# g1mv/density

Measured on NVIDIA H100. Metric: chameleon_encode_input_GBps, higher is better.
Workload: dtype u32

## Files before the change

density_b200/_lib.py:

```python
import ctypes
import os

_HERE = os.path.dirname(os.path.abspath(__file__))
SO_PATH = os.environ.get("DENSITY_B200_SO") or os.path.join(_HERE, "libdensity_b200.so")

_c_u8p = ctypes.c_void_p
_SIGS = {
    **{f"{a}_{op}": (ctypes.c_size_t, [_c_u8p, ctypes.c_size_t, _c_u8p, ctypes.c_size_t])
       for a in ("chameleon", "cheetah", "lion") for op in ("encode", "decode")},
    **{f"{a}_safe_encode_buffer_size": (ctypes.c_size_t, [ctypes.c_size_t]) for a in ("chameleon", "cheetah", "lion")},
    "density_b200_encode_device": (ctypes.c_int, [ctypes.c_int, _c_u8p, ctypes.c_size_t, _c_u8p, ctypes.c_size_t, ctypes.c_void_p, ctypes.c_void_p]),
    "density_b200_decode_device": (ctypes.c_int, [ctypes.c_int, _c_u8p, ctypes.c_size_t, _c_u8p, ctypes.c_size_t, ctypes.c_void_p, ctypes.c_void_p]),
    "density_b200_encode_device_path": (ctypes.c_int, [ctypes.c_int, _c_u8p, ctypes.c_size_t, _c_u8p, ctypes.c_size_t, ctypes.c_void_p, ctypes.c_void_p, ctypes.c_int]),
    "density_b200_decode_device_path": (ctypes.c_int, [ctypes.c_int, _c_u8p, ctypes.c_size_t, _c_u8p, ctypes.c_size_t, ctypes.c_void_p, ctypes.c_void_p, ctypes.c_int]),
    "density_b200_shard_create": (ctypes.c_void_p, []),
    "density_b200_shard_destroy": (None, [ctypes.c_void_p]),
    "density_b200_shard_phase1": (ctypes.c_int, [ctypes.c_void_p, _c_u8p, ctypes.c_size_t, ctypes.c_int, ctypes.c_void_p, ctypes.c_void_p]),
    "density_b200_shard_phase2": (ctypes.c_int, [ctypes.c_void_p, ctypes.c_void_p, _c_u8p, ctypes.c_size_t, ctypes.c_void_p, ctypes.c_void_p, ctypes.c_void_p]),
    "density_b200_sharded_unique_id": (ctypes.c_int, [ctypes.c_void_p]),
    "density_b200_sharded_create": (ctypes.c_void_p, [ctypes.c_void_p, ctypes.c_int, ctypes.c_int]),
    "density_b200_sharded_destroy": (None, [ctypes.c_void_p]),
    "density_b200_encode_sharded": (ctypes.c_int, [ctypes.c_void_p, _c_u8p, ctypes.c_size_t, _c_u8p, ctypes.c_size_t, ctypes.c_void_p, ctypes.c_void_p,
                                                   ctypes.c_void_p, ctypes.c_int, _c_u8p, ctypes.c_size_t, ctypes.c_void_p]),
    "density_b200_sharded_profile": (ctypes.c_int, [ctypes.c_void_p, ctypes.POINTER(ctypes.c_float)]),
# ... 23 lines not shown
    "density_b200_codec_create": (ctypes.c_void_p, [ctypes.c_int]),
    "density_b200_codec_destroy": (None, [ctypes.c_void_p]),
    "density_b200_codec_clear_state": (ctypes.c_int, [ctypes.c_void_p]),
    "density_b200_codec_encode": (ctypes.c_size_t, [ctypes.c_void_p, _c_u8p, ctypes.c_size_t, _c_u8p, ctypes.c_size_t]),
    "density_b200_codec_decode": (ctypes.c_size_t, [ctypes.c_void_p, _c_u8p, ctypes.c_size_t, _c_u8p, ctypes.c_size_t]),
    "density_b200_table_init": (ctypes.c_int, [ctypes.c_void_p, ctypes.c_void_p]),
    "density_b200_table_fold": (ctypes.c_int, [ctypes.c_void_p, ctypes.c_void_p, ctypes.c_void_p]),
    "density_b200_profile_enable": (None, [ctypes.c_int]),
    "density_b200_profile_get": (ctypes.c_int, [ctypes.POINTER(ctypes.c_float)]),
    "density_b200_last_error": (ctypes.c_char_p, []),
    "density_b200_kernel_launches": (ctypes.c_uint64, []),
    "density_b200_last_encode_was_fast": (ctypes.c_int, []),
    "density_b200_decode_status": (ctypes.c_int, [ctypes.POINTER(ctypes.c_uint64)]),
    "density_b200_cheetah_decode_rounds": (ctypes.c_int, [ctypes.POINTER(ctypes.c_uint32)]),
    "density_b200_encode_status": (ctypes.c_int, [ctypes.POINTER(ctypes.c_uint64)]),
    "density_b200_test_set_stage_rounds": (None, [ctypes.c_int]),
    "density_b200_prot_debug": (ctypes.c_int, [ctypes.POINTER(ctypes.c_uint64)]),
    "density_b200_shutdown": (None, []),
    "density_b200_version": (ctypes.c_char_p, []),
}
EXPORTED_SYMBOLS = tuple(sorted(_SIGS))

_lib = None


class DensityB200Error(RuntimeError):
    pass


def load():
# ... 18 lines not shown
```

density_b200/csrc/api.cu:

```cuda
#include "../../include/density_b200.h"
#include "common.cuh"
#include "encode_internal.cuh"

#include <dlfcn.h>

#include <atomic>
#include <condition_variable>
#include <cstdio>
#include <cstring>
#include <deque>
#include <mutex>
#include <string>
#include <thread>
#include <vector>

namespace dns {

static thread_local std::string g_last_error;
static std::atomic<uint64_t> g_launches{0};

static void set_error(const char* what, cudaError_t e) {
    char buf[512];
    snprintf(buf, sizeof buf, "%s: %s (%s)", what, cudaGetErrorString(e), cudaGetErrorName(e));
    g_last_error = buf;
// ... 137 lines not shown
struct DeviceCtx {
    int dev = -1;
    int num_sms = 0;
    bool ready = false;
    cudaStream_t stream = nullptr;
    cudaStream_t h2d_stream = nullptr, d2h_stream = nullptr;
    DevBuf ws, stage_in, stage_out, pipe_tables, dec_tables;
    DevBuf chee_tables[2][3];
    uint32_t chee_epoch = 0;
    uint64_t* h_sizes = nullptr;
    cudaEvent_t ev_h2d[2] = {nullptr, nullptr};
    PinRing ring_in, ring_out;
    uint64_t* d_size = nullptr;
    uint64_t* h_size = nullptr;
    ChamLayout layout{};
    int last_was_chameleon_fastpath_capable = 0;
    bool profile = false;
    static constexpr int PROF_RING = 64;
    cudaEvent_t ev[PROF_RING][4] = {};
    uint64_t prof_count = 0;
    const void* last_cl_status = nullptr;
    cudaEvent_t ws_free = nullptr;
    bool ws_free_recorded = false;
    std::mutex mu;
};

constexpr int MAX_DEVICES = 64;
static DeviceCtx g_ctx[MAX_DEVICES];
static std::mutex g_ctx_mu;

// ... 61 lines not shown
static int encode_device_locked_impl(DeviceCtx* c, int alg, const uint8_t* d_in, size_t n, uint8_t* d_out, size_t cap,
                                     uint64_t* d_out_size, cudaStream_t stream, int path) {
    uint64_t launches = 0;
    cudaError_t e;
    const bool aligned = !(reinterpret_cast<uintptr_t>(d_in) & 3) && !(reinterpret_cast<uintptr_t>(d_out) & 1);
    if (alg == ALG_CHAMELEON && path != 3 && aligned) {
        ChamLayout L;
        size_t need = cham_workspace_bytes(n, c->num_sms, &L);
        e = c->ws.ensure(need, stream);
        if (e != cudaSuccess) { set_error("workspace cudaMalloc", e); return DENSITY_B200_ECUDA; }
        c->layout = L;
        if (path == 2) {
            e = cham_encode_protected_only(d_in, n, c->ws.p, L, d_out, cap, d_out_size, stream, &launches);
        } else {
            const uint32_t nruns = cham_pick_runs(n, c->num_sms);
            cudaEvent_t* ev = nullptr;
            if (c->profile) {
                ev = c->ev[c->prof_count % DeviceCtx::PROF_RING];
                for (int i = 0; i < 4; ++i) if (!ev[i]) cudaEventCreate(&ev[i]);
            }
            e = cham_encode_phase1(d_in, n, c->ws.p, L, nruns, nullptr, stream, &launches, ev);
            if (e == cudaSuccess && path == 4)
                e = cham_encode_phase2_blocking(d_in, n, c->ws.p, L, nruns, d_out, cap, d_out_size, 12, stream, &launches);
            else if (e == cudaSuccess)
                e = cham_encode_phase2(d_in, n, c->ws.p, L, nruns, nullptr, d_out, cap, d_out_size, path == 0, false, stream, &launches, ev);
            if (ev != nullptr && e == cudaSuccess) c->prof_count++;
        }
        c->last_was_chameleon_fastpath_capable = (path != 2);
    } else if ((alg == ALG_CHEETAH || alg == ALG_LION) && path != 3 && !(reinterpret_cast<uintptr_t>(d_in) & 3) && !(reinterpret_cast<uintptr_t>(d_out) & 1)) {
        const size_t pw = (chee_workspace_bytes(n, c->num_sms) + 255) & ~(size_t)255;
// ... 1074 lines not shown
    if (cudaDeviceSynchronize() != cudaSuccess) return 0;
    if (cudaMemcpy(&st, c->ws.p + c->layout.status, sizeof st, cudaMemcpyDeviceToHost) != cudaSuccess) return 0;
    return st.nonquiet ? 0 : 1;
}

int density_b200_encode_status(uint64_t* out6) {
    DeviceCtx* c = current_ctx();
    if (!c || !c->ws.p) return DENSITY_B200_EARG;
    std::lock_guard<std::mutex> lk(c->mu);
    Status st;
    if (cudaDeviceSynchronize() != cudaSuccess || cudaMemcpy(&st, c->ws.p + c->layout.status, sizeof st, cudaMemcpyDeviceToHost) != cudaSuccess) return DENSITY_B200_ECUDA;
    out6[0] = st.out_bytes; out6[1] = st.nonquiet; out6[2] = st.error; out6[3] = st.first_nonquiet_block; out6[4] = st.converged; out6[5] = st.iter_changed;
    return DENSITY_B200_OK;
}

void density_b200_shutdown(void) {
    std::lock_guard<std::mutex> lk(g_ctx_mu);
    int cur = -1;
    cudaGetDevice(&cur);
    for (int d = 0; d < MAX_DEVICES; ++d) {
        DeviceCtx& c = g_ctx[d];
        if (!c.ready) continue;
        cudaSetDevice(d);
        c.ws.release(); c.stage_in.release(); c.stage_out.release(); c.dec_tables.release(); for (int a2 = 0; a2 < 2; ++a2) for (int rg = 0; rg < 3; ++rg) c.chee_tables[a2][rg].release();
        c.chee_epoch = 0;
        if (c.d_size) cudaFree(c.d_size);
        if (c.h_size) cudaFreeHost(c.h_size);
        if (c.stream) cudaStreamDestroy(c.stream);
        if (c.ws_free) { cudaEventDestroy(c.ws_free); c.ws_free = nullptr; c.ws_free_recorded = false; }
        if (c.h2d_stream) cudaStreamDestroy(c.h2d_stream);
// ... 32 lines not shown
```

density_b200/csrc/chameleon_encode.cu:

```cuda
#include <cstdio>
#include "common.cuh"
#include "encode_internal.cuh"

namespace dns {
namespace cham {

constexpr int TILE_Q = 4096;
__device__ __forceinline__ bool bit_test(const uint32_t* bm, uint32_t i) { return (bm[i >> 5] >> (i & 31)) & 1u; }

constexpr int F6_THREADS = 512, F6_QPT = 8;
constexpr int F6_NW = F6_THREADS / 32, F6_WQ = 32 * F6_QPT;
static_assert(F6_THREADS * F6_QPT == TILE_Q, "tile geometry");
constexpr int F6_MB_SLOTS = 4096, F6_MB_CAP = 4;
constexpr int F6_SEC_SLOTS = 64, F6_SEC_CAP = 16;
#ifdef DNS_PHASE_TIMING
__device__ long long g_f6_ph[8];
#define F6_PH(k) { if (threadIdx.x == 0 && blockIdx.x == 77) { long long tn = clock64(); g_f6_ph[k] += tn - f6_tprev; f6_tprev = tn; } }
#define F6_PH_DECL long long f6_tprev = clock64();
#else
#define F6_PH(k)
#define F6_PH_DECL
#endif
constexpr uint32_t F6_TOUCHED = 1u << 12, F6_DROPPED = 1u << 13;
struct Flag6Smem {
// ... 334 lines not shown
        const uint32_t v = S.tab[i];
        const uint32_t tch = (v != 0 || bit_test(S.vbit, i)) ? 0x10000u : 0u;
        final_tab[(size_t)run * 65536 + i] = v | tch;
    }
    if (tid == 0) unres_count[run] = S.unres_count < 65536u ? S.unres_count : 65536u;
#ifdef DNS_PHASE_TIMING
    if (tid == 0 && run == 77 && ntile_run) { const long long nt = ntile_run;
        printf("f6 run %u tiles %lld cycles/tile: A %lld B %lld C+deposit %lld D+S4 %lld  overflow tiles %lld dirty/tile %lld\n", run, nt, g_f6_ph[0] / nt, g_f6_ph[1] / nt,
               g_f6_ph[2] / nt, g_f6_ph[3] / nt, g_f6_ph[6], g_f6_ph[7] / nt);
        for (int k = 0; k < 8; ++k) g_f6_ph[k] = 0; }
#endif
}

__device__ __forceinline__ bool gate_open(const Status* g) { return !g || (g->nonquiet && !g->converged); }

__global__ void cham_carry_scan(const uint32_t* __restrict__ final_tab, const uint32_t* __restrict__ init, int init_untouched,
                                uint32_t nruns, uint32_t* __restrict__ carry, uint32_t* __restrict__ table_out,
                                const Status* __restrict__ gate = nullptr) {
    if (!gate_open(gate)) return;
    uint32_t hb = blockIdx.x * blockDim.x + threadIdx.x;
    if (hb >= 65536) return;
    uint32_t c = init ? init[hb] : ((hb == 0 && !init_untouched) ? 0x10000u : 0u);
    for (uint32_t r = 0; r < nruns; ++r) {
        if (carry) carry[(size_t)r * 65536 + hb] = c;
        uint32_t v = final_tab[(size_t)r * 65536 + hb];
        if (v & 0x10000u) c = v;
    }
    if (table_out) table_out[hb] = c;
}

__global__ void cham_resolve(const uint2* __restrict__ unres, const uint32_t* __restrict__ unres_count,
                             const uint32_t* __restrict__ carry, uint32_t tiles_total, uint32_t nruns,
                             uint32_t* __restrict__ sigw_g, const Status* __restrict__ gate = nullptr) {
    if (!gate_open(gate)) return;
    const uint32_t run = blockIdx.y;
    const uint32_t n = unres_count[run];
    const uint64_t run_q0 = ((uint64_t)run * tiles_total / nruns) * TILE_Q;
    for (uint32_t i = blockIdx.x * blockDim.x + threadIdx.x; i < n; i += gridDim.x * blockDim.x) {
        uint2 e = unres[(size_t)run * 65536 + i];
        uint32_t c = carry[(size_t)run * 65536 + (e.y & 0xFFFFu)];
        if ((c & 0x10000u) && (c & 0xFFFFu) == (e.y >> 16)) {
            uint64_t gq = run_q0 + e.x;
            atomicOr(&sigw_g[gq >> 5], 1u << (gq & 31));
        }
    }
}

struct ProtSmem {
    uint16_t tab[65536];
    uint32_t vbit[2048];
};

__global__ void __launch_bounds__(1024, 1)
cham_protected_pass(const uint32_t* __restrict__ in, uint64_t nbytes, const Status* __restrict__ status, int only_if_nonquiet,
                    uint32_t* __restrict__ sigw_g, uint8_t* __restrict__ copymap) {
    if (only_if_nonquiet && !(status->nonquiet && !status->converged)) return;
    extern __shared__ __align__(16) unsigned char smem_raw[];
    ProtSmem& S = *reinterpret_cast<ProtSmem*>(smem_raw);
// ... 270 lines not shown
        for (uint64_t b = gtid; b < nblocks; b += gsz) cm_old[b] = __ldcg(&cm_new[b]);
    grid_barrier(bar, gridDim.x, epoch);
    if (gtid == 0 && converged) st->converged = 1;
}

__device__ __forceinline__ uint32_t block_out_bytes(uint64_t b, uint64_t nbytes, uint32_t hits, bool copied) {
    const uint64_t boff = b * 256;
    const uint32_t blen = (uint32_t)((nbytes - boff < 256) ? (nbytes - boff) : 256);
    return copied ? blen : 8 + blen - 2 * hits;
}

__global__ void cham_tile_sizes(const uint32_t* __restrict__ sigw_g, const uint8_t* __restrict__ copymap, uint64_t nbytes,
                                uint64_t nblocks, uint32_t ntiles, int use_copymap_if_nonquiet, int check_quiet, int assume_prev_inc,
                                Status* __restrict__ status, uint32_t* __restrict__ tile_bytes) {
    const uint32_t lane = threadIdx.x & 31;
    const uint32_t tile = blockIdx.x * (blockDim.x >> 5) + (threadIdx.x >> 5);
    if (tile >= ntiles) return;
    if (use_copymap_if_nonquiet && !check_quiet && !status->nonquiet) return;
    const bool use_cm = copymap && (!use_copymap_if_nonquiet || status->nonquiet);
    uint32_t sum = 0, incm[2];
#pragma unroll
    for (int k = 0; k < 2; ++k) {
        const uint64_t b = (uint64_t)tile * 64 + k * 32 + lane;
        uint32_t sz = 0; bool inc = false;
        if (b < nblocks) {
            const bool copied = use_cm && copymap[b];
            const uint32_t hits = __popc(sigw_g[2 * b]) + __popc(sigw_g[2 * b + 1]);
            sz = block_out_bytes(b, nbytes, hits, copied);
            inc = !copied && sz >= 256 && (nbytes - b * 256 >= 256);
        }
        sum += sz;
        incm[k] = __ballot_sync(0xFFFFFFFFu, inc);
    }
#pragma unroll
    for (int d = 16; d; d >>= 1) sum += __shfl_xor_sync(0xFFFFFFFFu, sum, d);
    if (lane == 0) tile_bytes[tile] = sum;
    if (check_quiet && lane == 0) {
        bool prev = assume_prev_inc != 0;
        if (tile > 0) {
            const uint64_t b = (uint64_t)tile * 64 - 1;
            const uint32_t hits = __popc(sigw_g[2 * b]) + __popc(sigw_g[2 * b + 1]);
            prev = (8 + 256 - 2 * hits) >= 256;
        }
        const uint64_t m = ((uint64_t)incm[1] << 32) | incm[0];
        const uint64_t pairs = m & ((m << 1) | (prev ? 1ull : 0ull));
        if (pairs) {
            atomicOr(&status->nonquiet, 1u);
            atomicMin(&status->first_nonquiet_block, (unsigned long long)tile * 64 + (__ffsll((long long)pairs) - 1));
        }
    }
}

constexpr int SCAN_T = 1024;
constexpr int SCAN_PER = 4;
constexpr int SCAN_G = SCAN_T * SCAN_PER;

__device__ __forceinline__ uint64_t block_exclusive_scan_u64(uint64_t v, uint64_t* s_warp, uint64_t* total) {
    const uint32_t lane = threadIdx.x & 31, warp = threadIdx.x >> 5;
    uint64_t incl = v;
#pragma unroll
    for (int d = 1; d < 32; d <<= 1) { uint64_t u = __shfl_up_sync(0xFFFFFFFFu, incl, d); if (lane >= (uint32_t)d) incl += u; }
    if (lane == 31) s_warp[warp] = incl;
    __syncthreads();
// ... 255 lines not shown
        if (w[2]) bad = 1;
        if (w[3]) { if (prev_inc && w[0]) bad = 1; prev_inc = w[1]; }
        if (d_sizes) d_sizes[r] = off;
        off += (uint64_t)w[4] | ((uint64_t)w[5] << 32);
    }
    if (d_sizes) d_sizes[world] = off;
    if (d_flags) *d_flags = bad;
    if (d_total) *d_total = off;
    (void)rank;
}

}

using namespace cham;

size_t cham_workspace_bytes(size_t nbytes, int nruns_max, ChamLayout* L) {
    const uint64_t nblocks = (nbytes + 255) / 256;
    const uint64_t ntiles = (nblocks + 63) / 64;
    const uint64_t ngroups = (ntiles + SCAN_G - 1) / SCAN_G;
    size_t off = 0;
    auto take = [&](size_t bytes) { size_t o = off; off += (bytes + 255) & ~(size_t)255; return o; };
    L->status = take(sizeof(Status));
    L->sigw = take((ntiles * 64 * 2 + 64 + 256) * sizeof(uint32_t));
    L->copymap = take(ntiles * 64 + 64 + 128);
    L->copymap2 = take(ntiles * 64 + 64 + 128);
    L->seg_state = take(prot_state_bytes(ntiles * 64 / PSEG + 2));
    L->incb = take(ntiles * 64 + 64);
    L->tile_bytes = take((ntiles + 1) * sizeof(uint32_t));
    L->tile_local = take((ntiles + 1) * sizeof(uint32_t));
    L->group_total = take((ngroups + 1) * sizeof(uint64_t));
    L->group_off = take((ngroups + 1) * sizeof(uint64_t));
    L->unres = take((size_t)nruns_max * 65536 * sizeof(uint2));
    L->unres_count = take((size_t)nruns_max * sizeof(uint32_t));
    L->final_tab = take((size_t)nruns_max * 65536 * sizeof(uint32_t));
    L->carry = take((size_t)nruns_max * 65536 * sizeof(uint32_t));
    L->total = off;
    return off;
}

static cudaError_t set_smem_attrs_once() {
    static bool done = false;
    static cudaError_t err = cudaSuccess;
    if (!done) {
        err = cudaFuncSetAttribute(cham_flag_pass6, cudaFuncAttributeMaxDynamicSharedMemorySize, (int)sizeof(Flag6Smem));
        if (err == cudaSuccess)
            err = cudaFuncSetAttribute(cham_protected_pass, cudaFuncAttributeMaxDynamicSharedMemorySize, (int)sizeof(ProtSmem));
        done = true;
    }
    return err;
}

static void launch_flag_pass(uint32_t nruns, cudaStream_t stream, const uint32_t* in, uint64_t nquads, uint32_t ntiles, uint32_t* sigw,
                             uint2* unres, uint32_t* unres_count, uint32_t* final_tab, const uint8_t* copymap, const Status* gate) {
    cham_flag_pass6<<<nruns, F6_THREADS, sizeof(Flag6Smem), stream>>>(in, nquads, ntiles, nruns, sigw, unres, unres_count, final_tab, copymap, gate);
}

static cudaError_t prot_iterate_coop(int ctas, cudaStream_t stream, const uint32_t* sigw, uint64_t nbytes, uint64_t nblocks, uint32_t nseg, Status* st, int it,
                                     uint8_t* inc, uint8_t* cm_old, uint8_t* cm_new, uint32_t* in_state, uint32_t* out_state, uint16_t* ptab) {
    void* args[] = {&sigw, &nbytes, &nblocks, &nseg, &st, &it, &inc, &cm_old, &cm_new, &in_state, &out_state, &ptab};
    return cudaLaunchCooperativeKernel(reinterpret_cast<const void*>(prot_iterate), dim3((unsigned)ctas), dim3(PI_THREADS), args, 0, stream);
}

cudaError_t prot_debug_read(unsigned long long* out32) { return cudaMemcpyFromSymbol(out32, g_prot_dbg, sizeof(unsigned long long) * 32); }

size_t prot_state_bytes(uint64_t nseg_max) { return (2 * (nseg_max + 2) + 64) * sizeof(uint32_t) + prot_table_elems(nseg_max) * sizeof(uint16_t); }

uint32_t cham_pick_runs(size_t nbytes, int num_sms) {
    const uint64_t nblocks = (nbytes + 255) / 256;
    const uint64_t ntiles = (nblocks + 63) / 64;
// ... 13 lines not shown
    Status* st = reinterpret_cast<Status*>(ws + L.status);
    e = cudaMemsetAsync(st, 0, sizeof(Status), stream);
    if (e != cudaSuccess) return e;
    {
        e = cudaMemsetAsync(&st->first_nonquiet_block, 0xFF, sizeof(unsigned long long), stream);
        if (e != cudaSuccess) return e;
    }
    if (nblocks == 0) return cudaSuccess;
    if (ev) cudaEventRecord(ev[0], stream);
    launch_flag_pass(nruns, stream, reinterpret_cast<const uint32_t*>(d_in), nquads, ntiles, reinterpret_cast<uint32_t*>(ws + L.sigw),
        reinterpret_cast<uint2*>(ws + L.unres), reinterpret_cast<uint32_t*>(ws + L.unres_count),
        reinterpret_cast<uint32_t*>(ws + L.final_tab), nullptr, nullptr);
    ++*launches;
    if (ev) cudaEventRecord(ev[1], stream);
    if (d_table_out) {
        cham_carry_scan<<<65536 / 256, 256, 0, stream>>>(reinterpret_cast<uint32_t*>(ws + L.final_tab), nullptr, 1, nruns,
                                                        nullptr, d_table_out);
        ++*launches;
    }
    return cudaGetLastError();
}

cudaError_t cham_phase2_begin(const uint8_t* d_in, size_t nbytes, uint8_t* ws, const ChamLayout& L, uint32_t nruns, const uint32_t* d_carry_in,
                              bool assume_prev_inc, cudaStream_t stream, uint64_t* launches) {
    (void)d_in;
    const uint64_t nblocks = (nbytes + 255) / 256;
    const uint32_t ntiles = (uint32_t)((nblocks + 63) / 64);
    Status* st = reinterpret_cast<Status*>(ws + L.status);
    uint32_t* sigw = reinterpret_cast<uint32_t*>(ws + L.sigw);
    cham_carry_scan<<<65536 / 256, 256, 0, stream>>>(reinterpret_cast<uint32_t*>(ws + L.final_tab), d_carry_in, 0, nruns,
                                                    reinterpret_cast<uint32_t*>(ws + L.carry), nullptr);
    cham_resolve<<<dim3(32, nruns), 256, 0, stream>>>(reinterpret_cast<uint2*>(ws + L.unres), reinterpret_cast<uint32_t*>(ws + L.unres_count),
                                                     reinterpret_cast<uint32_t*>(ws + L.carry), ntiles, nruns, sigw);
    cham_tile_sizes<<<(ntiles + 7) / 8, 256, 0, stream>>>(sigw, nullptr, nbytes, nblocks, ntiles, 0, 1, assume_prev_inc ? 1 : 0, st,
                                                          reinterpret_cast<uint32_t*>(ws + L.tile_bytes));
    *launches += 3;
    return cudaGetLastError();
}

cudaError_t cham_phase2_rounds(const uint8_t* d_in, size_t nbytes, uint8_t* ws, const ChamLayout& L, uint32_t nruns, const uint32_t* d_carry_in,
                               int it_first, int it_last, bool reset_barriers, cudaStream_t stream, uint64_t* launches) {
    const uint64_t nblocks = (nbytes + 255) / 256;
    const uint32_t ntiles = (uint32_t)((nblocks + 63) / 64);
    Status* st = reinterpret_cast<Status*>(ws + L.status);
    uint32_t* sigw = reinterpret_cast<uint32_t*>(ws + L.sigw);
    uint8_t* copymap = ws + L.copymap;
    uint8_t* copymap2 = ws + L.copymap2;
    uint32_t* seg_state = reinterpret_cast<uint32_t*>(ws + L.seg_state);
    uint8_t* incb = ws + L.incb;
    int num_ctas = 0;
    { int dev = 0; cudaGetDevice(&dev); cudaDeviceGetAttribute(&num_ctas, cudaDevAttrMultiProcessorCount, dev); if (num_ctas < 1) num_ctas = 1; }
    const uint32_t nseg = (uint32_t)((nblocks + PSEG - 1) / PSEG);
    const uint32_t* in32 = reinterpret_cast<const uint32_t*>(d_in);
    const uint64_t nquads = nbytes / 4;
    if (it_last - it_first >= 8) return cudaErrorInvalidValue;
    if (reset_barriers) {
        cudaError_t e = cudaMemsetAsync(st->barrier, 0, sizeof(st->barrier), stream);
        if (e != cudaSuccess) return e;
    }
    for (int it = it_first; it <= it_last; ++it) {
        if (it > 0) {
            launch_flag_pass(nruns, stream, in32, nquads, ntiles, sigw,
                reinterpret_cast<uint2*>(ws + L.unres), reinterpret_cast<uint32_t*>(ws + L.unres_count),
                reinterpret_cast<uint32_t*>(ws + L.final_tab), copymap, st);
            cham_carry_scan<<<65536 / 256, 256, 0, stream>>>(reinterpret_cast<uint32_t*>(ws + L.final_tab), d_carry_in, 0, nruns,
                                                            reinterpret_cast<uint32_t*>(ws + L.carry), nullptr, st);
            cham_resolve<<<dim3(32, nruns), 256, 0, stream>>>(reinterpret_cast<uint2*>(ws + L.unres), reinterpret_cast<uint32_t*>(ws + L.unres_count),
                                                             reinterpret_cast<uint32_t*>(ws + L.carry), ntiles, nruns, sigw, st);
            *launches += 3;
        }
        {
            cudaError_t le = prot_iterate_coop(num_ctas, stream, sigw, nbytes, nblocks, nseg, st, it, incb, copymap, copymap2, seg_state, seg_state + (nseg + 1),
                                               reinterpret_cast<uint16_t*>(seg_state + 2 * (nseg + 1)));
            if (le != cudaSuccess) return le;
        }
        ++*launches;
    }
    return cudaGetLastError();
}

cudaError_t cham_phase2_finish(const uint8_t* d_in, size_t nbytes, uint8_t* ws, const ChamLayout& L, uint8_t* d_out, size_t cap,
                               uint64_t* d_out_size, bool with_copy_map, cudaStream_t stream, uint64_t* launches, cudaEvent_t* ev,
                               bool inorder_fallback = true) {
    const uint64_t nblocks = (nbytes + 255) / 256;
    const uint32_t ntiles = (uint32_t)((nblocks + 63) / 64);
    const uint32_t ngroups = (ntiles + SCAN_G - 1) / SCAN_G;
    Status* st = reinterpret_cast<Status*>(ws + L.status);
    uint32_t* sigw = reinterpret_cast<uint32_t*>(ws + L.sigw);
    uint8_t* copymap = ws + L.copymap;
    if (with_copy_map) {
        if (inorder_fallback) { cham_protected_pass<<<1, 1024, sizeof(ProtSmem), stream>>>(reinterpret_cast<const uint32_t*>(d_in), nbytes, st, 1, sigw, copymap); ++*launches; }
        cham_tile_sizes<<<(ntiles + 7) / 8, 256, 0, stream>>>(sigw, copymap, nbytes, nblocks, ntiles, 1, 0, 0, st,
                                                              reinterpret_cast<uint32_t*>(ws + L.tile_bytes));
        ++*launches;
    }
    scan_groups_local<<<ngroups, SCAN_T, 0, stream>>>(reinterpret_cast<uint32_t*>(ws + L.tile_bytes), ntiles,
                                                      reinterpret_cast<uint32_t*>(ws + L.tile_local),
                                                      reinterpret_cast<uint64_t*>(ws + L.group_total));
    scan_group_totals<<<1, SCAN_T, 0, stream>>>(reinterpret_cast<uint64_t*>(ws + L.group_total), ngroups,
                                                reinterpret_cast<uint64_t*>(ws + L.group_off), st, (uint64_t)cap, d_out_size);
    *launches += 2;
    if (ev) cudaEventRecord(ev[2], stream);
    if ((reinterpret_cast<uintptr_t>(d_in) & 15u) == 0)
        cham_emit<true><<<ntiles, EM_THREADS, 0, stream>>>(reinterpret_cast<const uint32_t*>(d_in), nbytes, nblocks, sigw,
                                                           with_copy_map ? copymap : nullptr, 1, st,
                                                           reinterpret_cast<uint32_t*>(ws + L.tile_local),
                                                           reinterpret_cast<uint64_t*>(ws + L.group_off), d_out);
// ... 50 lines not shown
                                      uint64_t* launches, bool* ok) {
    *ok = true;
    if (nbytes == 0) return cudaMemsetAsync(d_out_size, 0, sizeof(uint64_t), stream);
    cudaError_t e = cham_phase2_begin(d_in, nbytes, ws, L, nruns, d_carry_in, false, stream, launches);
    if (e == cudaSuccess) e = cham_phase2_rounds(d_in, nbytes, ws, L, nruns, d_carry_in, 0, PROT_ITERS, false, stream, launches);
    bool more = false;
    for (int batch = 0; e == cudaSuccess; ++batch) {
        e = cham_phase2_needs_more(ws, L, stream, &more);
        if (e != cudaSuccess || !more || batch >= max_batches) break;
        e = cham_phase2_rounds(d_in, nbytes, ws, L, nruns, d_carry_in, 8, 15, true, stream, launches);
    }
    if (e != cudaSuccess) return e;
    if (more) { *ok = false; return cudaSuccess; }
    e = cham_phase2_finish(d_in, nbytes, ws, L, d_out, cap, d_out_size, true, stream, launches, nullptr, false);
    if (e == cudaSuccess) {
        cham_carry_scan<<<65536 / 256, 256, 0, stream>>>(reinterpret_cast<uint32_t*>(ws + L.final_tab), nullptr, 1, nruns, nullptr, d_table_out);
        ++*launches;
        e = cudaGetLastError();
    }
    return e;
}
cudaError_t cham_quads_to_table(const uint32_t* d_quads, uint32_t* d_table, cudaStream_t stream, uint64_t* launches) {
    cham_quads_to_table_k<<<65536 / 256, 256, 0, stream>>>(d_quads, d_table);
    ++*launches;
    return cudaGetLastError();
}
cudaError_t cham_table_into_quads(const uint32_t* d_table, uint32_t* d_quads, cudaStream_t stream, uint64_t* launches) {
    cham_table_into_quads_k<<<65536 / 256, 256, 0, stream>>>(d_table, d_quads);
    ++*launches;
    return cudaGetLastError();
}
// ... 49 lines not shown
cudaError_t cham_encode_protected_only(const uint8_t* d_in, size_t nbytes, uint8_t* ws, const ChamLayout& L, uint8_t* d_out,
                                       size_t cap, uint64_t* d_out_size, cudaStream_t stream, uint64_t* launches) {
    cudaError_t e = set_smem_attrs_once();
    if (e != cudaSuccess) return e;
    const uint64_t nblocks = (nbytes + 255) / 256;
    const uint32_t ntiles = (uint32_t)((nblocks + 63) / 64);
    const uint32_t ngroups = (ntiles + SCAN_G - 1) / SCAN_G;
    Status* st = reinterpret_cast<Status*>(ws + L.status);
    uint32_t* sigw = reinterpret_cast<uint32_t*>(ws + L.sigw);
    uint8_t* copymap = ws + L.copymap;
    e = cudaMemsetAsync(st, 0, sizeof(Status), stream);
    if (e != cudaSuccess) return e;
    if (nblocks == 0) return cudaMemsetAsync(d_out_size, 0, sizeof(uint64_t), stream);
    cham_protected_pass<<<1, 1024, sizeof(ProtSmem), stream>>>(reinterpret_cast<const uint32_t*>(d_in), nbytes, st, 0, sigw, copymap);
    ++*launches;
    cham_tile_sizes<<<(ntiles + 7) / 8, 256, 0, stream>>>(sigw, copymap, nbytes, nblocks, ntiles, 0, 0, 0, st,
                                                          reinterpret_cast<uint32_t*>(ws + L.tile_bytes));
    ++*launches;
    scan_groups_local<<<ngroups, SCAN_T, 0, stream>>>(reinterpret_cast<uint32_t*>(ws + L.tile_bytes), ntiles,
                                                      reinterpret_cast<uint32_t*>(ws + L.tile_local),
                                                      reinterpret_cast<uint64_t*>(ws + L.group_total));
    ++*launches;
    scan_group_totals<<<1, SCAN_T, 0, stream>>>(reinterpret_cast<uint64_t*>(ws + L.group_total), ngroups,
                                                reinterpret_cast<uint64_t*>(ws + L.group_off), st, (uint64_t)cap, d_out_size);
    ++*launches;
    cham_emit<false><<<ntiles, EM_THREADS, 0, stream>>>(reinterpret_cast<const uint32_t*>(d_in), nbytes, nblocks, sigw, copymap, 0, st,
                                                        reinterpret_cast<uint32_t*>(ws + L.tile_local),
                                                        reinterpret_cast<uint64_t*>(ws + L.group_off), d_out);
    ++*launches;
    return cudaGetLastError();
}
// ... 3 lines not shown
```

density_b200/csrc/encode_internal.cuh:

```cuda
#pragma once
#include <cuda_runtime.h>
#include <stdint.h>
#include <stddef.h>

namespace dns {

struct ChamLayout {
    size_t status, sigw, copymap, copymap2, seg_state, incb, tile_bytes, tile_local, group_total, group_off, unres, unres_count, final_tab, carry, total;
};

size_t cham_workspace_bytes(size_t nbytes, int nruns_max, ChamLayout* L);
uint32_t cham_pick_runs(size_t nbytes, int num_sms);
cudaError_t cham_encode_phase1(const uint8_t* d_in, size_t nbytes, uint8_t* ws, const ChamLayout& L, uint32_t nruns,
                               uint32_t* d_table_out, cudaStream_t stream, uint64_t* launches, cudaEvent_t* ev = nullptr);
cudaError_t cham_encode_phase2(const uint8_t* d_in, size_t nbytes, uint8_t* ws, const ChamLayout& L, uint32_t nruns,
                               const uint32_t* d_carry_in, uint8_t* d_out, size_t cap, uint64_t* d_out_size,
                               bool allow_protected_fallback, bool assume_prev_inc, cudaStream_t stream, uint64_t* launches,
                               cudaEvent_t* ev = nullptr);
cudaError_t cham_encode_phase2_blocking(const uint8_t* d_in, size_t nbytes, uint8_t* ws, const ChamLayout& L, uint32_t nruns, uint8_t* d_out,
                                        size_t cap, uint64_t* d_out_size, int max_batches, cudaStream_t stream, uint64_t* launches);
cudaError_t cham_encode_protected_only(const uint8_t* d_in, size_t nbytes, uint8_t* ws, const ChamLayout& L, uint8_t* d_out,
                                       size_t cap, uint64_t* d_out_size, cudaStream_t stream, uint64_t* launches);

cudaError_t cham_quads_to_table(const uint32_t* d_quads, uint32_t* d_table, cudaStream_t stream, uint64_t* launches);
// ... 73 lines not shown
```

include/density_b200.h:

```cpp
#ifndef DENSITY_B200_H
#define DENSITY_B200_H

#include <stddef.h>
#include <stdint.h>

#if defined(__GNUC__)
#define DENSITY_B200_API __attribute__((visibility("default")))
#else
#define DENSITY_B200_API
#endif

#ifdef __cplusplus
extern "C" {
#endif

DENSITY_B200_API size_t chameleon_encode(const uint8_t* input, size_t input_size, uint8_t* output, size_t output_size);
DENSITY_B200_API size_t chameleon_decode(const uint8_t* input, size_t input_size, uint8_t* output, size_t output_size);
DENSITY_B200_API size_t chameleon_safe_encode_buffer_size(size_t size);

DENSITY_B200_API size_t cheetah_encode(const uint8_t* input, size_t input_size, uint8_t* output, size_t output_size);
DENSITY_B200_API size_t cheetah_decode(const uint8_t* input, size_t input_size, uint8_t* output, size_t output_size);
DENSITY_B200_API size_t cheetah_safe_encode_buffer_size(size_t size);

DENSITY_B200_API size_t lion_encode(const uint8_t* input, size_t input_size, uint8_t* output, size_t output_size);
// ... 5 lines not shown
#define DENSITY_B200_LION 2

#define DENSITY_B200_OK 0
#define DENSITY_B200_ECUDA 1
#define DENSITY_B200_ECAPACITY 2
#define DENSITY_B200_EMALFORMED 3
#define DENSITY_B200_EARG 4

DENSITY_B200_API int density_b200_encode_device(int alg, const uint8_t* d_in, size_t n, uint8_t* d_out, size_t cap,
                               uint64_t* d_out_size, void* stream);
DENSITY_B200_API int density_b200_encode_device_path(int alg, const uint8_t* d_in, size_t n, uint8_t* d_out, size_t cap,
                                    uint64_t* d_out_size, void* stream, int path);
DENSITY_B200_API int density_b200_decode_device_path(int alg, const uint8_t* d_in, size_t n, uint8_t* d_out, size_t cap,
                                    uint64_t* d_out_size, void* stream, int path);
DENSITY_B200_API int density_b200_encode_status(uint64_t* out6);
DENSITY_B200_API int density_b200_decode_status(uint64_t* out10);
DENSITY_B200_API int density_b200_cheetah_decode_rounds(uint32_t* out4);
DENSITY_B200_API int density_b200_decode_device(int alg, const uint8_t* d_in, size_t n, uint8_t* d_out, size_t cap,
                               uint64_t* d_out_size, void* stream);

typedef struct density_b200_shard density_b200_shard;
DENSITY_B200_API density_b200_shard* density_b200_shard_create(void);
DENSITY_B200_API void density_b200_shard_destroy(density_b200_shard*);
DENSITY_B200_API int density_b200_shard_phase1(density_b200_shard*, const uint8_t* d_in, size_t n, int is_last_shard,
                              uint32_t* d_table_out, void* stream);
DENSITY_B200_API int density_b200_shard_phase2(density_b200_shard*, const uint32_t* d_carry_in, uint8_t* d_out, size_t cap,
                              uint64_t* d_out_size, uint32_t* d_flags, void* stream);
DENSITY_B200_API int density_b200_table_init(uint32_t* d_table, void* stream);
DENSITY_B200_API int density_b200_table_fold(uint32_t* d_acc, const uint32_t* d_next, void* stream);

// ... 66 lines not shown
```

Measured before the change: 480.9.

## Replace per-run carry table with grouped carry and warp-aggregated resolve walk

Replaces the full per-run carry scan, which wrote a 65536-entry carry array for every run, with a coarse carry snapshot every 16 runs. Each unresolved entry now walks back through final_tab within its group to find its carry. Bit sets are merged across the warp with match_any/reduce_or so fewer atomics are issued. It also caps the tile_sizes grid at 8 blocks per SM using a grid-stride loop, and adds a debug API that reads back unresolved counts. The cost is extra random reads per unresolved entry during the walk, plus a device-attribute query on each launch.

```diff
diff --git a/density_b200/_lib.py b/density_b200/_lib.py
--- a/density_b200/_lib.py
+++ b/density_b200/_lib.py
@@ -61,6 +61,7 @@
     "density_b200_decode_status": (ctypes.c_int, [ctypes.POINTER(ctypes.c_uint64)]),
     "density_b200_cheetah_decode_rounds": (ctypes.c_int, [ctypes.POINTER(ctypes.c_uint32)]),
     "density_b200_encode_status": (ctypes.c_int, [ctypes.POINTER(ctypes.c_uint64)]),
+    "density_b200_encode_unresolved": (ctypes.c_int, [ctypes.POINTER(ctypes.c_uint32), ctypes.c_int, ctypes.POINTER(ctypes.c_int)]),
     "density_b200_test_set_stage_rounds": (None, [ctypes.c_int]),
     "density_b200_prot_debug": (ctypes.c_int, [ctypes.POINTER(ctypes.c_uint64)]),
     "density_b200_shutdown": (None, []),
diff --git a/density_b200/csrc/api.cu b/density_b200/csrc/api.cu
--- a/density_b200/csrc/api.cu
+++ b/density_b200/csrc/api.cu
@@ -175,6 +175,7 @@
     uint64_t* d_size = nullptr;
     uint64_t* h_size = nullptr;
     ChamLayout layout{};
+    uint32_t last_nruns = 0;
     int last_was_chameleon_fastpath_capable = 0;
     bool profile = false;
     static constexpr int PROF_RING = 64;
@@ -266,6 +267,7 @@
             e = cham_encode_protected_only(d_in, n, c->ws.p, L, d_out, cap, d_out_size, stream, &launches);
         } else {
             const uint32_t nruns = cham_pick_runs(n, c->num_sms);
+            c->last_nruns = nruns;
             cudaEvent_t* ev = nullptr;
             if (c->profile) {
                 ev = c->ev[c->prof_count % DeviceCtx::PROF_RING];
@@ -1370,6 +1372,18 @@
     return DENSITY_B200_OK;
 }
 
+int density_b200_encode_unresolved(uint32_t* out, int cap, int* nruns) {
+    DeviceCtx* c = current_ctx();
+    if (!c || !c->ws.p || !out || !nruns || cap < 0) return DENSITY_B200_EARG;
+    std::lock_guard<std::mutex> lk(c->mu);
+    if (c->last_was_chameleon_fastpath_capable != 1) return DENSITY_B200_EARG;
+    *nruns = (int)c->last_nruns;
+    const size_t k = c->last_nruns < (uint32_t)cap ? c->last_nruns : (uint32_t)cap;
+    if (cudaDeviceSynchronize() != cudaSuccess ||
+        cudaMemcpy(out, c->ws.p + c->layout.unres_count, k * sizeof(uint32_t), cudaMemcpyDeviceToHost) != cudaSuccess) return DENSITY_B200_ECUDA;
+    return DENSITY_B200_OK;
+}
+
 void density_b200_shutdown(void) {
     std::lock_guard<std::mutex> lk(g_ctx_mu);
     int cur = -1;
diff --git a/density_b200/csrc/chameleon_encode.cu b/density_b200/csrc/chameleon_encode.cu
--- a/density_b200/csrc/chameleon_encode.cu
+++ b/density_b200/csrc/chameleon_encode.cu
@@ -372,34 +372,67 @@
 
 __device__ __forceinline__ bool gate_open(const Status* g) { return !g || (g->nonquiet && !g->converged); }
 
-__global__ void cham_carry_scan(const uint32_t* __restrict__ final_tab, const uint32_t* __restrict__ init, int init_untouched,
-                                uint32_t nruns, uint32_t* __restrict__ carry, uint32_t* __restrict__ table_out,
-                                const Status* __restrict__ gate = nullptr) {
-    if (!gate_open(gate)) return;
+__global__ void cham_carry_scan(const uint32_t* __restrict__ final_tab, uint32_t nruns, uint32_t* __restrict__ table_out) {
     uint32_t hb = blockIdx.x * blockDim.x + threadIdx.x;
     if (hb >= 65536) return;
-    uint32_t c = init ? init[hb] : ((hb == 0 && !init_untouched) ? 0x10000u : 0u);
+    uint32_t c = 0;
     for (uint32_t r = 0; r < nruns; ++r) {
-        if (carry) carry[(size_t)r * 65536 + hb] = c;
         uint32_t v = final_tab[(size_t)r * 65536 + hb];
         if (v & 0x10000u) c = v;
     }
-    if (table_out) table_out[hb] = c;
-}
-
-__global__ void cham_resolve(const uint2* __restrict__ unres, const uint32_t* __restrict__ unres_count,
-                             const uint32_t* __restrict__ carry, uint32_t tiles_total, uint32_t nruns,
-                             uint32_t* __restrict__ sigw_g, const Status* __restrict__ gate = nullptr) {
+    table_out[hb] = c;
+}
+
+constexpr uint32_t RES_G = 16;
+
+__global__ void cham_group_carry(const uint32_t* __restrict__ final_tab, const uint32_t* __restrict__ init, uint32_t nruns,
+                                 uint32_t* __restrict__ gcarry, const Status* __restrict__ gate = nullptr) {
     if (!gate_open(gate)) return;
-    const uint32_t run = blockIdx.y;
+    const uint32_t hb = blockIdx.x * blockDim.x + threadIdx.x;
+    if (hb >= 65536) return;
+    uint32_t c = init ? init[hb] : (hb == 0 ? 0x10000u : 0u);
+    for (uint32_t g = 0;; ++g) {
+        gcarry[(size_t)g * 65536 + hb] = c;
+        const uint32_t r0 = g * RES_G;
+        if (r0 + RES_G >= nruns) break;
+        uint32_t v[RES_G];
+#pragma unroll
+        for (uint32_t k = 0; k < RES_G; ++k) v[k] = final_tab[(size_t)(r0 + k) * 65536 + hb];
+#pragma unroll
+        for (uint32_t k = 0; k < RES_G; ++k) if (v[k] & 0x10000u) c = v[k];
+    }
+}
+
+__global__ void cham_resolve_walk(const uint2* __restrict__ unres, const uint32_t* __restrict__ unres_count,
+                                  const uint32_t* __restrict__ final_tab, const uint32_t* __restrict__ gcarry, uint32_t tiles_total,
+                                  uint32_t nruns, uint32_t* __restrict__ sigw_g, const Status* __restrict__ gate = nullptr) {
+    if (!gate_open(gate)) return;
+    const uint32_t run = blockIdx.y, lane = threadIdx.x & 31;
     const uint32_t n = unres_count[run];
-    const uint64_t run_q0 = ((uint64_t)run * tiles_total / nruns) * TILE_Q;
-    for (uint32_t i = blockIdx.x * blockDim.x + threadIdx.x; i < n; i += gridDim.x * blockDim.x) {
-        uint2 e = unres[(size_t)run * 65536 + i];
-        uint32_t c = carry[(size_t)run * 65536 + (e.y & 0xFFFFu)];
-        if ((c & 0x10000u) && (c & 0xFFFFu) == (e.y >> 16)) {
-            uint64_t gq = run_q0 + e.x;
-            atomicOr(&sigw_g[gq >> 5], 1u << (gq & 31));
+    const uint32_t g = run / RES_G, r_first = g * RES_G;
+    uint32_t* __restrict__ rsig = sigw_g + ((uint64_t)run * tiles_total / nruns) * (TILE_Q / 32);
+    const uint2* __restrict__ list = unres + (size_t)run * 65536;
+    for (uint32_t base = (blockIdx.x * blockDim.x + threadIdx.x) & ~31u; base < n; base += gridDim.x * blockDim.x) {
+        const uint32_t i = base + lane;
+        bool hit = false;
+        uint2 e = make_uint2(0, 0);
+        if (i < n) {
+            e = list[i];
+            const uint32_t h = e.y & 0xFFFFu;
+            uint32_t c = 0;
+            uint32_t r = run;
+            for (; r > r_first; --r) {
+                c = final_tab[(size_t)(r - 1) * 65536 + h];
+                if (c & 0x10000u) break;
+            }
+            if (r == r_first) c = gcarry[(size_t)g * 65536 + h];
+            hit = (c & 0x10000u) && (c & 0xFFFFu) == (e.y >> 16);
+        }
+        const uint32_t hm = __ballot_sync(0xFFFFFFFFu, hit);
+        if (hit) {
+            const uint32_t peers = __match_any_sync(hm, e.x >> 5);
+            const uint32_t bits = __reduce_or_sync(peers, 1u << (e.x & 31));
+            if (lane == (uint32_t)__ffs(peers) - 1u) atomicOr(&rsig[e.x >> 5], bits);
         }
     }
 }
@@ -700,39 +733,39 @@
                                 uint64_t nblocks, uint32_t ntiles, int use_copymap_if_nonquiet, int check_quiet, int assume_prev_inc,
                                 Status* __restrict__ status, uint32_t* __restrict__ tile_bytes) {
     const uint32_t lane = threadIdx.x & 31;
-    const uint32_t tile = blockIdx.x * (blockDim.x >> 5) + (threadIdx.x >> 5);
-    if (tile >= ntiles) return;
     if (use_copymap_if_nonquiet && !check_quiet && !status->nonquiet) return;
     const bool use_cm = copymap && (!use_copymap_if_nonquiet || status->nonquiet);
-    uint32_t sum = 0, incm[2];
-#pragma unroll
-    for (int k = 0; k < 2; ++k) {
-        const uint64_t b = (uint64_t)tile * 64 + k * 32 + lane;
-        uint32_t sz = 0; bool inc = false;
-        if (b < nblocks) {
-            const bool copied = use_cm && copymap[b];
-            const uint32_t hits = __popc(sigw_g[2 * b]) + __popc(sigw_g[2 * b + 1]);
-            sz = block_out_bytes(b, nbytes, hits, copied);
-            inc = !copied && sz >= 256 && (nbytes - b * 256 >= 256);
-        }
-        sum += sz;
-        incm[k] = __ballot_sync(0xFFFFFFFFu, inc);
-    }
-#pragma unroll
-    for (int d = 16; d; d >>= 1) sum += __shfl_xor_sync(0xFFFFFFFFu, sum, d);
-    if (lane == 0) tile_bytes[tile] = sum;
-    if (check_quiet && lane == 0) {
-        bool prev = assume_prev_inc != 0;
-        if (tile > 0) {
-            const uint64_t b = (uint64_t)tile * 64 - 1;
-            const uint32_t hits = __popc(sigw_g[2 * b]) + __popc(sigw_g[2 * b + 1]);
-            prev = (8 + 256 - 2 * hits) >= 256;
-        }
-        const uint64_t m = ((uint64_t)incm[1] << 32) | incm[0];
-        const uint64_t pairs = m & ((m << 1) | (prev ? 1ull : 0ull));
-        if (pairs) {
-            atomicOr(&status->nonquiet, 1u);
-            atomicMin(&status->first_nonquiet_block, (unsigned long long)tile * 64 + (__ffsll((long long)pairs) - 1));
+    for (uint32_t tile = blockIdx.x * (blockDim.x >> 5) + (threadIdx.x >> 5); tile < ntiles; tile += gridDim.x * (blockDim.x >> 5)) {
+        uint32_t sum = 0, incm[2];
+    #pragma unroll
+        for (int k = 0; k < 2; ++k) {
+            const uint64_t b = (uint64_t)tile * 64 + k * 32 + lane;
+            uint32_t sz = 0; bool inc = false;
+            if (b < nblocks) {
+                const bool copied = use_cm && copymap[b];
+                const uint32_t hits = __popc(sigw_g[2 * b]) + __popc(sigw_g[2 * b + 1]);
+                sz = block_out_bytes(b, nbytes, hits, copied);
+                inc = !copied && sz >= 256 && (nbytes - b * 256 >= 256);
+            }
+            sum += sz;
+            incm[k] = __ballot_sync(0xFFFFFFFFu, inc);
+        }
+    #pragma unroll
+        for (int d = 16; d; d >>= 1) sum += __shfl_xor_sync(0xFFFFFFFFu, sum, d);
+        if (lane == 0) tile_bytes[tile] = sum;
+        if (check_quiet && lane == 0) {
+            bool prev = assume_prev_inc != 0;
+            if (tile > 0) {
+                const uint64_t b = (uint64_t)tile * 64 - 1;
+                const uint32_t hits = __popc(sigw_g[2 * b]) + __popc(sigw_g[2 * b + 1]);
+                prev = (8 + 256 - 2 * hits) >= 256;
+            }
+            const uint64_t m = ((uint64_t)incm[1] << 32) | incm[0];
+            const uint64_t pairs = m & ((m << 1) | (prev ? 1ull : 0ull));
+            if (pairs) {
+                atomicOr(&status->nonquiet, 1u);
+                atomicMin(&status->first_nonquiet_block, (unsigned long long)tile * 64 + (__ffsll((long long)pairs) - 1));
+            }
         }
     }
 }
@@ -1018,6 +1051,13 @@
 
 using namespace cham;
 
+static unsigned tile_sizes_grid(uint32_t ntiles) {
+    int dev = 0, sms = 0;
+    cudaGetDevice(&dev); cudaDeviceGetAttribute(&sms, cudaDevAttrMultiProcessorCount, dev);
+    const uint32_t want = (ntiles + 7) / 8, cap = 8u * (uint32_t)(sms > 0 ? sms : 1);
+    return want < cap ? want : cap;
+}
+
 size_t cham_workspace_bytes(size_t nbytes, int nruns_max, ChamLayout* L) {
     const uint64_t nblocks = (nbytes + 255) / 256;
     const uint64_t ntiles = (nblocks + 63) / 64;
@@ -1037,7 +1077,7 @@
     L->unres = take((size_t)nruns_max * 65536 * sizeof(uint2));
     L->unres_count = take((size_t)nruns_max * sizeof(uint32_t));
     L->final_tab = take((size_t)nruns_max * 65536 * sizeof(uint32_t));
-    L->carry = take((size_t)nruns_max * 65536 * sizeof(uint32_t));
+    L->gcarry = take((size_t)((nruns_max + RES_G - 1) / RES_G) * 65536 * sizeof(uint32_t));
     L->total = off;
     return off;
 }
@@ -1057,6 +1097,16 @@
 static void launch_flag_pass(uint32_t nruns, cudaStream_t stream, const uint32_t* in, uint64_t nquads, uint32_t ntiles, uint32_t* sigw,
                              uint2* unres, uint32_t* unres_count, uint32_t* final_tab, const uint8_t* copymap, const Status* gate) {
     cham_flag_pass6<<<nruns, F6_THREADS, sizeof(Flag6Smem), stream>>>(in, nquads, ntiles, nruns, sigw, unres, unres_count, final_tab, copymap, gate);
+}
+
+static void launch_resolve(uint32_t nruns, uint32_t ntiles, uint8_t* ws, const ChamLayout& L, const uint32_t* d_carry_in, uint32_t* sigw,
+                           const Status* gate, cudaStream_t stream) {
+    const uint32_t* final_tab = reinterpret_cast<const uint32_t*>(ws + L.final_tab);
+    uint32_t* gcarry = reinterpret_cast<uint32_t*>(ws + L.gcarry);
+    cham_group_carry<<<65536 / 256, 256, 0, stream>>>(final_tab, d_carry_in, nruns, gcarry, gate);
+    cham_resolve_walk<<<dim3(32, nruns), 256, 0, stream>>>(reinterpret_cast<const uint2*>(ws + L.unres),
+                                                          reinterpret_cast<const uint32_t*>(ws + L.unres_count), final_tab, gcarry, ntiles,
+                                                          nruns, sigw, gate);
 }
 
 static cudaError_t prot_iterate_coop(int ctas, cudaStream_t stream, const uint32_t* sigw, uint64_t nbytes, uint64_t nblocks, uint32_t nseg, Status* st, int it,
@@ -1100,8 +1150,7 @@
     ++*launches;
     if (ev) cudaEventRecord(ev[1], stream);
     if (d_table_out) {
-        cham_carry_scan<<<65536 / 256, 256, 0, stream>>>(reinterpret_cast<uint32_t*>(ws + L.final_tab), nullptr, 1, nruns,
-                                                        nullptr, d_table_out);
+        cham_carry_scan<<<65536 / 256, 256, 0, stream>>>(reinterpret_cast<uint32_t*>(ws + L.final_tab), nruns, d_table_out);
         ++*launches;
     }
     return cudaGetLastError();
@@ -1114,11 +1163,8 @@
     const uint32_t ntiles = (uint32_t)((nblocks + 63) / 64);
     Status* st = reinterpret_cast<Status*>(ws + L.status);
     uint32_t* sigw = reinterpret_cast<uint32_t*>(ws + L.sigw);
-    cham_carry_scan<<<65536 / 256, 256, 0, stream>>>(reinterpret_cast<uint32_t*>(ws + L.final_tab), d_carry_in, 0, nruns,
-                                                    reinterpret_cast<uint32_t*>(ws + L.carry), nullptr);
-    cham_resolve<<<dim3(32, nruns), 256, 0, stream>>>(reinterpret_cast<uint2*>(ws + L.unres), reinterpret_cast<uint32_t*>(ws + L.unres_count),
-                                                     reinterpret_cast<uint32_t*>(ws + L.carry), ntiles, nruns, sigw);
-    cham_tile_sizes<<<(ntiles + 7) / 8, 256, 0, stream>>>(sigw, nullptr, nbytes, nblocks, ntiles, 0, 1, assume_prev_inc ? 1 : 0, st,
+    launch_resolve(nruns, ntiles, ws, L, d_carry_in, sigw, nullptr, stream);
+    cham_tile_sizes<<<tile_sizes_grid(ntiles), 256, 0, stream>>>(sigw, nullptr, nbytes, nblocks, ntiles, 0, 1, assume_prev_inc ? 1 : 0, st,
                                                           reinterpret_cast<uint32_t*>(ws + L.tile_bytes));
     *launches += 3;
     return cudaGetLastError();
@@ -1149,10 +1195,7 @@
             launch_flag_pass(nruns, stream, in32, nquads, ntiles, sigw,
                 reinterpret_cast<uint2*>(ws + L.unres), reinterpret_cast<uint32_t*>(ws + L.unres_count),
                 reinterpret_cast<uint32_t*>(ws + L.final_tab), copymap, st);
-            cham_carry_scan<<<65536 / 256, 256, 0, stream>>>(reinterpret_cast<uint32_t*>(ws + L.final_tab), d_carry_in, 0, nruns,
-                                                            reinterpret_cast<uint32_t*>(ws + L.carry), nullptr, st);
-            cham_resolve<<<dim3(32, nruns), 256, 0, stream>>>(reinterpret_cast<uint2*>(ws + L.unres), reinterpret_cast<uint32_t*>(ws + L.unres_count),
-                                                             reinterpret_cast<uint32_t*>(ws + L.carry), ntiles, nruns, sigw, st);
+            launch_resolve(nruns, ntiles, ws, L, d_carry_in, sigw, st, stream);
             *launches += 3;
         }
         {
@@ -1176,7 +1219,7 @@
     uint8_t* copymap = ws + L.copymap;
     if (with_copy_map) {
         if (inorder_fallback) { cham_protected_pass<<<1, 1024, sizeof(ProtSmem), stream>>>(reinterpret_cast<const uint32_t*>(d_in), nbytes, st, 1, sigw, copymap); ++*launches; }
-        cham_tile_sizes<<<(ntiles + 7) / 8, 256, 0, stream>>>(sigw, copymap, nbytes, nblocks, ntiles, 1, 0, 0, st,
+        cham_tile_sizes<<<tile_sizes_grid(ntiles), 256, 0, stream>>>(sigw, copymap, nbytes, nblocks, ntiles, 1, 0, 0, st,
                                                               reinterpret_cast<uint32_t*>(ws + L.tile_bytes));
         ++*launches;
     }
@@ -1257,7 +1300,7 @@
     if (more) { *ok = false; return cudaSuccess; }
     e = cham_phase2_finish(d_in, nbytes, ws, L, d_out, cap, d_out_size, true, stream, launches, nullptr, false);
     if (e == cudaSuccess) {
-        cham_carry_scan<<<65536 / 256, 256, 0, stream>>>(reinterpret_cast<uint32_t*>(ws + L.final_tab), nullptr, 1, nruns, nullptr, d_table_out);
+        cham_carry_scan<<<65536 / 256, 256, 0, stream>>>(reinterpret_cast<uint32_t*>(ws + L.final_tab), nruns, d_table_out);
         ++*launches;
         e = cudaGetLastError();
     }
@@ -1337,7 +1380,7 @@
     if (nblocks == 0) return cudaMemsetAsync(d_out_size, 0, sizeof(uint64_t), stream);
     cham_protected_pass<<<1, 1024, sizeof(ProtSmem), stream>>>(reinterpret_cast<const uint32_t*>(d_in), nbytes, st, 0, sigw, copymap);
     ++*launches;
-    cham_tile_sizes<<<(ntiles + 7) / 8, 256, 0, stream>>>(sigw, copymap, nbytes, nblocks, ntiles, 0, 0, 0, st,
+    cham_tile_sizes<<<tile_sizes_grid(ntiles), 256, 0, stream>>>(sigw, copymap, nbytes, nblocks, ntiles, 0, 0, 0, st,
                                                           reinterpret_cast<uint32_t*>(ws + L.tile_bytes));
     ++*launches;
     scan_groups_local<<<ngroups, SCAN_T, 0, stream>>>(reinterpret_cast<uint32_t*>(ws + L.tile_bytes), ntiles,
diff --git a/density_b200/csrc/encode_internal.cuh b/density_b200/csrc/encode_internal.cuh
--- a/density_b200/csrc/encode_internal.cuh
+++ b/density_b200/csrc/encode_internal.cuh
@@ -6,7 +6,7 @@
 namespace dns {
 
 struct ChamLayout {
-    size_t status, sigw, copymap, copymap2, seg_state, incb, tile_bytes, tile_local, group_total, group_off, unres, unres_count, final_tab, carry, total;
+    size_t status, sigw, copymap, copymap2, seg_state, incb, tile_bytes, tile_local, group_total, group_off, unres, unres_count, final_tab, gcarry, total;
 };
 
 size_t cham_workspace_bytes(size_t nbytes, int nruns_max, ChamLayout* L);
diff --git a/include/density_b200.h b/include/density_b200.h
--- a/include/density_b200.h
+++ b/include/density_b200.h
@@ -43,6 +43,7 @@
 DENSITY_B200_API int density_b200_decode_device_path(int alg, const uint8_t* d_in, size_t n, uint8_t* d_out, size_t cap,
                                     uint64_t* d_out_size, void* stream, int path);
 DENSITY_B200_API int density_b200_encode_status(uint64_t* out6);
+DENSITY_B200_API int density_b200_encode_unresolved(uint32_t* out, int cap, int* nruns);
 DENSITY_B200_API int density_b200_decode_status(uint64_t* out10);
 DENSITY_B200_API int density_b200_cheetah_decode_rounds(uint32_t* out4);
 DENSITY_B200_API int density_b200_decode_device(int alg, const uint8_t* d_in, size_t n, uint8_t* d_out, size_t cap,
```

Result: no change. 485.2 (median of 6 runs) (+0.9%).
